# yongduosui/CAL

Measured on AMD Instinct MI355X. Metric: graphs/sec (train step) on SPMotif b=0.9 batch=128, higher is better.
Workload: dtype f32; 1 GPU; spmotif_b0.9_causalgcn_h128_l3_bs128; model=CausalGCN, batch_per_gpu=128, global_batch=128, hidden=128, layers=3, node_num=7, launch=graph(8 steps per graph launch, remainder 3), parallelism=dp1, resident_batches=8

## Files before the change

### cal_amd/csrc/engine.hip

```cpp
#include <string.h>
#include <hip/hip_ext.h>

#include <algorithm>
#include <type_traits>
#include <vector>

#include "engine_kernels.hpp"
#include "engine_readout.hpp"
#include "engine_gconv.hpp"
#include "engine_gconv_bwd.hpp"
#include "engine_ggat.hpp"
#include "engine_plan.hpp"
#include "engine_attbwd.hpp"
#include "engine_ro_step.hpp"
#include "engine_gin.hpp"
#include "engine_ggin.hpp"
#include "engine_feat.hpp"
#include "engine_gwide.hpp"
#include "engine_attwide.hpp"

namespace cal {

constexpr int MAX_LAYERS = 6;
constexpr int MAX_SLABS = 24;
// ... 1035 lines not shown
            { ProfScope ps(st, 0, 2.0 * N * H * H); RC(fwd_gemm(c, false, a, 1)); } STAGE();
            {
                ProfScope ps(st, 5, 2.0 * N * H * 4 + (double)(E + N) * (8 + 12.0 * K) + (N + 1) * 4.0);
                RC(gat_forward(e->rowptr_dst, e->nbr_dst, e->eid_dst, zi, e->P + e->o_conv_att[i - 1], e->P + e->o_conv_b[i - 1], 1,
                               e->gat_slope, c.training ? e->gat_p : 0.f, e->gat_seed[i - 1], (const uint64_t*)e->gat_ctr, hout,
                               sc, sc + nk, sc + 2 * nk, sc + 3 * nk, N, E, K, D, st));
            }
            STAGE();
            if (c.training && i < L) {
                int tc = std::min(256, pow2ceil(H));
                int rpb = std::max(32, cdiv(N, 1024));
                if (H == 256 && aligned16(hout))
                    hipLaunchKernelGGL(k_colstats4, dim3(cdiv(N, rpb)), dim3(256), 0, st, hout, N, rpb, Acc(bn_stsum(c, i + 1)), Acc(bn_stsq(c, i + 1)));
                else
                    hipLaunchKernelGGL(k_colstats, dim3(cdiv(N, rpb)), dim3(256), 0, st, hout, N, H, tc, rpb, Acc(bn_stsum(c, i + 1)), Acc(bn_stsq(c, i + 1)));
                CAL_CHECK_LAUNCH("k_colstats"); STAGE();
            }
        } else if (r.bb_fwd != Conv::Node) {
            GconvBranch gb;
            memset(&gb, 0, sizeof(gb));
            gb.x = hin; gb.W = e->P + e->o_conv_w[i - 1]; gb.bias = e->P + e->o_conv_b[i - 1];
            gb.dis = e->dis_unit; gb.bn = bnref(c, i, N, 1); gb.out = hout;
            if (i == 1 && !r.plan_coef) gb.coef_out = e->coef; else gb.coef_in = e->coef;
            if (c.training && i < L) { gb.st_sum = graph_acc(c, bn_stsum(c, i + 1), H, r.st_bb); gb.st_sq = graph_acc(c, bn_stsq(c, i + 1), H, r.st_bb); }
            const GconvBranch2 b2{{gb, gb}};
            {
                ProfScope ps(st, 2, 2.0 * N * H * H + 2.0 * (double)(E + N) * H, true);
                if (r.bb_fwd == Conv::Wide && r.gw_cols_bb == 32) PROF_LAUNCH((k_gw_fwd<false, 32>), dim3(T, H / 32, 1), dim3(GW_NT), 0, st, gd, e->gptr, e->eptr, b2, 1, e->loop_w, H, H, e->status);
                else if (r.bb_fwd == Conv::Wide) PROF_LAUNCH((k_gw_fwd<false, 64>), dim3(T, H / GC_N, 1), dim3(GW_NT), 0, st, gd, e->gptr, e->eptr, b2, 1, e->loop_w, H, H, e->status);
                else if (r.bb_fwd == Conv::Graph64) PROF_LAUNCH((k_gconv_fwd<false, 64, 512>), dim3(T, H / GC_N, 1), dim3(512), 0, st, gd, e->gptr, e->eptr, b2, 1, e->loop_w, H, H, e->status);
                else PROF_LAUNCH((k_gconv_fwd<false, GC_T>), dim3(T, H / GC_N, 1), dim3(256), 0, st, gd, e->gptr, e->eptr, b2, 1, e->loop_w, H, H, e->status);
            }
            CAL_CHECK_LAUNCH(r.bb_fwd == Conv::Wide ? "k_gw_fwd" : "k_gconv_fwd"); STAGE();
            RC(flush_finals(c)); STAGE();
        } else {
            GemmArgs a = gemm_args(N, H, H, false, false, 0);
            a.p[0].A = hin; a.p[0].B = e->P + e->o_conv_w[i - 1]; a.p[0].C = e->z;
            a.p[0].xa.has_bn = 1; a.p[0].xa.bn = bnref(c, i, N, 1);
            { ProfScope ps(st, 0, 2.0 * N * H * H); RC(fwd_gemm(c, false, a, 1)); } STAGE();
            SpmmBranch br{e->z, hout, e->P + e->o_conv_b[i - 1], nullptr, e->dis_unit, Acc(), Acc(), nullptr, nullptr, nullptr};
            const bool wst = c.training && i < L;
            const int rpb = spmm_rpb(H, wst, N);
            if (wst) { br.st_sum = spmm_acc(c, bn_stsum(c, i + 1), H, rpb); br.st_sq = spmm_acc(c, bn_stsq(c, i + 1), H, rpb); }
            {
                ProfScope ps(st, 1, 2.0 * N * H * 4 + (double)(E + N) * 8 + (N + 1) * 4.0, true);
                RC(launch_espmm(st, gd, SpmmBranch2{{br, br}}, 1, 1, e->loop_w, N, H, rpb));
            }
            CAL_CHECK_LAUNCH("k_espmm"); STAGE();
            RC(flush_finals(c)); STAGE();
        }
    }
    return 0;
}

int fwd_att(Ctx& c) {
    Engine* e = c.e;
    const Route& r = c.r;
    const int N = c.N, H = e->H, L = e->L;
    const int64_t E = c.E;
    hipStream_t st = c.st;
    const float* x = e->h + (size_t)L * N * H;
    const CSR gs = csr_src(c);
    if (r.att_fwd != Att::Node) {
        const bool wide = r.att_fwd == Att::Wide;
        const Acc a0 = graph_acc(c, bn_stsum(c, L + 1), H, r.st_co), a1 = graph_acc(c, bn_stsq(c, L + 1), H, r.st_co);
        const Acc a2 = graph_acc(c, bn_stsum(c, L + 2), H, r.st_co), a3 = graph_acc(c, bn_stsq(c, L + 2), H, r.st_co);
        auto launch = [&](auto kernel_of) {
            return with_g(H, [&](auto g) {
                hipLaunchKernelGGL(kernel_of(g), dim3(c.T), dim3(512), 0, st, e->gptr, gs, x, e->P + e->o_natt_w, e->P + e->o_natt_b,
                                   e->P + e->o_eatt_w, e->P + e->o_eatt_b, e->anode, e->pq, e->att, e->dis_co, e->dis_co + N, a0, a1, a2, a3,
                                   e->loop_w, H, E, e->status, e->no_node_att ? 0.f : 1.f, e->no_edge_att ? 0.f : 1.f, e->eptr);
                return 0;
            });
        };
        if (wide) RC(launch([](auto g) { return k_att_fwd_wide<4, decltype(g)::value>; }));
        else RC(launch([](auto g) { return k_att_fwd_graph<4, decltype(g)::value>; }));
        CAL_CHECK_LAUNCH(wide ? "k_att_fwd_wide" : "k_att_fwd_graph"); STAGE();
        RC(flush_finals(c)); STAGE();
        return 0;
    }
    const Acc a0 = node_acc(c, bn_stsum(c, L + 1), H), a1 = node_acc(c, bn_stsq(c, L + 1), H);
    const Acc a2 = node_acc(c, bn_stsum(c, L + 2), H), a3 = node_acc(c, bn_stsq(c, L + 2), H);
    RC(with_g(H, [&](auto g) {
        constexpr int G = decltype(g)::value;
        hipLaunchKernelGGL((k_node_att_fwd<4, G>), dim3(cdiv(N, c.rpb_n)), dim3(256), 0, st, x, e->P + e->o_natt_w,
                           e->P + e->o_natt_b, e->P + e->o_eatt_w, e->anode, e->pq, a0, a1, a2, a3, N, H, c.rpb_n, e->no_node_att ? 0.f : 1.f);
        return 0;
    }));
    CAL_CHECK_LAUNCH("k_node_att_fwd"); STAGE();
    RC(flush_finals(c)); STAGE();
    hipLaunchKernelGGL(k_edge_att_deg, dim3(cdiv(N, 32)), dim3(256), 0, st, gs, e->pq, e->P + e->o_eatt_b, e->att, e->dis_co,
                       e->dis_co + N, e->loop_w, N, E, e->no_edge_att ? 0.f : 1.f);
    CAL_CHECK_LAUNCH("k_edge_att_deg"); STAGE();
    return 0;
}

int fwd_co(Ctx& c) {
    Engine* e = c.e;
    const Route& r = c.r;
    const int N = c.N, B = c.B, T = c.T, H = e->H, L = e->L;
    const int64_t E = c.E;
    hipStream_t st = c.st;
    const size_t NH = (size_t)N * H;
    const float* x = e->h + (size_t)L * NH;
    const CSR gd = csr_dst(c);
    if (r.co_fwd != Conv::Node) {
        const bool wide = r.co_fwd == Conv::Wide;
        const int64_t* tgp = e->ntiles > 0 ? e->tile_gptr : nullptr;
        GconvBranch gb[2];
        memset(gb, 0, sizeof(gb));
        for (int k = 0; k < 2; ++k) {
            gb[k].x = x; gb[k].W = e->P + (k ? e->o_ow : e->o_cw); gb[k].bias = e->P + (k ? e->o_ob : e->o_cb);
            gb[k].ew = e->att + (size_t)k * E; gb[k].dis = e->dis_co + (size_t)k * N;
            gb[k].rs = e->anode + k; gb[k].rs_stride = 2; gb[k].bn = bnref(c, L + 1 + k, N, 1);
            gb[k].out = e->hco + (size_t)k * NH; gb[k].z = e->zco + (size_t)k * NH; gb[k].pooled = e->pooled + (size_t)k * B * H;
            if (wide) continue;
            gb[k].coef_out = e->coef + (size_t)(1 + k) * E;
            gb[k].w_out = e->wslot + (size_t)k * E;
            gb[k].batch = c.batch; gb[k].tile_gptr = tgp;
        }
        const GconvBranch2 b2{{gb[0], gb[1]}};
        if (tgp) hipLaunchKernelGGL((k_gconv_fwd<true, 64, 512, true>), dim3(T, H / GC_N, 2), dim3(512), 0, st, gd, e->gptr, e->eptr, b2, 1, e->loop_w, H, H, e->status);
        else if (r.co_fwd == Conv::Graph64) hipLaunchKernelGGL((k_gconv_fwd<true, 64, 512>), dim3(T, H / GC_N, 2), dim3(512), 0, st, gd, e->gptr, e->eptr, b2, 1, e->loop_w, H, H, e->status);
        else if (r.co_fwd == Conv::Graph128) hipLaunchKernelGGL((k_gconv_fwd<true, GC_T>), dim3(T, H / GC_N, 2), dim3(256), 0, st, gd, e->gptr, e->eptr, b2, 1, e->loop_w, H, H, e->status);
        else if (r.gw_cols_co == 32) hipLaunchKernelGGL((k_gw_fwd<true, 32>), dim3(T, H / 32, 2), dim3(GW_NT), 0, st, gd, e->gptr, e->eptr, b2, 1, e->loop_w, H, H, e->status);
        else hipLaunchKernelGGL((k_gw_fwd<true, 64>), dim3(T, H / GC_N, 2), dim3(GW_NT), 0, st, gd, e->gptr, e->eptr, b2, 1, e->loop_w, H, H, e->status);
        CAL_CHECK_LAUNCH(wide ? "k_gw_fwd(co)" : "k_gconv_fwd(co)"); STAGE();
        return 0;
    }
    GemmArgs a = gemm_args(N, H, H, false, false, 0);
    for (int k = 0; k < 2; ++k) {
        a.p[k].A = x; a.p[k].B = e->P + (k ? e->o_ow : e->o_cw); a.p[k].C = e->zco + (size_t)k * NH;
        a.p[k].xa.rs = e->anode + k; a.p[k].xa.rs_stride = 2;
        a.p[k].xa.has_bn = 1; a.p[k].xa.bn = bnref(c, L + 1 + k, N, 1);
    }
    RC(fwd_gemm(c, false, a, 2)); STAGE();
    SpmmBranch b0{e->zco, e->hco, e->P + e->o_cb, e->att, e->dis_co, Acc(), Acc(), nullptr, nullptr, nullptr};
    SpmmBranch b1{e->zco + NH, e->hco + NH, e->P + e->o_ob, e->att + E, e->dis_co + N, Acc(), Acc(), nullptr, nullptr, nullptr};
    RC(launch_espmm(st, gd, SpmmBranch2{{b0, b1}}, 2, 1, e->loop_w, N, H, spmm_rpb(H, false)));
    CAL_CHECK_LAUNCH("k_espmm(co)"); STAGE();
    RC(launch_pool2(c)); STAGE();
    return 0;
}

int fwd_readout(Ctx& c) {
    Engine* e = c.e;
    const int B = c.B, H = e->H, C = e->C, L = e->L;
    hipStream_t st = c.st;
    if (c.r.ro == Readout::OneLaunch || c.r.ro == Readout::Rows) {
        RoStepArgs sa;
        memset(&sa, 0, sizeof(sa));
        sa.a = make_ro(c); sa.zpart = e->zpart; sa.sync = reinterpret_cast<int*>(e->arena + e->a_sync); sa.status = e->status;
        if (c.r.ro == Readout::OneLaunch) {
            hipLaunchKernelGGL(k_ro_step<false>, dim3(3, H / RO_CW), dim3(256), 0, st, sa);
        } else {
            const int nrb = cdiv(B, RS_B), nch = H / RO_CW;
            sa.nrb = nrb;
            sa.xch = parts_alloc(c, (size_t)3 * nch * RBK_XCH);
            if (!sa.xch) return no_parts();
            sa.gw1_slab = e->slabs; sa.gw2_slab = e->slabs + (size_t)3 * nrb * H * H;
            hipLaunchKernelGGL(k_ro_step<true>, dim3(3, nch, nrb), dim3(256), 0, st, sa);
        }
        CAL_CHECK_LAUNCH("k_ro_step"); STAGE();
        return 0;
    }
    if (c.r.ro == Readout::FourKernel) {
        const RoArgs ra = make_ro(c);
        hipLaunchKernelGGL(k_ro_fwd_a, dim3(3, H / RO_CW), dim3(256), 0, st, ra);
        CAL_CHECK_LAUNCH("k_ro_fwd_a"); STAGE();
        hipLaunchKernelGGL(k_ro_fwd_b, dim3(3, cdiv(B, RO_RB)), dim3(256), 0, st, ra);
        CAL_CHECK_LAUNCH("k_ro_fwd_b"); STAGE();
        if (!c.want_grad) {
            hipLaunchKernelGGL(k_ro_loss, dim3(3), dim3(256), 0, st, ra);
            CAL_CHECK_LAUNCH("k_ro_loss");
        }
        return 0;
    }
    const int bn_fc1 = L + 3, bn_fc2 = L + 4;
    {
        int tc = std::min(256, pow2ceil(H));
        hipLaunchKernelGGL(k_readout_prep, dim3(cdiv(B, c.rpb_b)), dim3(256), 0, st, e->pooled, c.perm, e->iperm, e->xco, B, H, tc,
                           c.rpb_b, bn_stsum(c, bn_fc1), bn_stsq(c, bn_fc1), bn_stsum(c, bn_fc1 + 2), bn_stsq(c, bn_fc1 + 2),
                           bn_stsum(c, bn_fc1 + 4), bn_stsq(c, bn_fc1 + 4), e->cat);
        CAL_CHECK_LAUNCH("k_readout_prep"); STAGE();
    }
    const float* xin[3] = {e->pooled, e->pooled + (size_t)B * H, e->xco};
    const int Wco = e->cat ? 2 * H : H;
    {
        auto fc1 = [&](int hd0, int nh, int Kin) -> int {
            GemmArgs a = gemm_args(B, H, Kin, false, true, 1);
            for (int q = 0; q < nh; ++q) {
                const int hd = hd0 + q;
                a.p[q].A = xin[hd]; a.p[q].B = e->P + e->o_fc1_w[hd]; a.p[q].bias = e->P + e->o_fc1_b[hd];
                a.p[q].C = e->y1 + (size_t)hd * B * H;
                a.p[q].xa.has_bn = 1; a.p[q].xa.bn = bnref(c, bn_fc1 + 2 * hd, B, 1);
                if (c.training) gemm_stats(c, a.p[q], B, H, bn_stsum(c, bn_fc2 + 2 * hd), bn_stsq(c, bn_fc2 + 2 * hd), false);
            }
            return fwd_gemm(c, true, a, nh);
        };
        if (e->cat) { RC(fc1(0, 2, H)); STAGE(); RC(fc1(2, 1, Wco)); STAGE(); }
        else { RC(fc1(0, 3, H)); STAGE(); }
        RC(flush_finals(c)); STAGE();
    }
    {
        GemmArgs a = gemm_args(B, C, H, false, true, 0);
        for (int hd = 0; hd < 3; ++hd) {
            a.p[hd].A = e->y1 + (size_t)hd * B * H; a.p[hd].B = e->P + e->o_fc2_w[hd]; a.p[hd].bias = e->P + e->o_fc2_b[hd];
            a.p[hd].C = e->zl + (size_t)hd * B * C;
            a.p[hd].xa.has_bn = 1; a.p[hd].xa.bn = bnref(c, bn_fc2 + 2 * hd, B, 1);
        }
        RC(fwd_gemm(c, true, a, 3)); STAGE();
    }
    if (B > 256) hipLaunchKernelGGL(k_loss<1024>, dim3(1), dim3(1024), 0, st, e->zl, c.y, e->logp, e->dzl, e->stats, e->arena + e->a_db2, B, C, c.wc, c.wo,
                                    c.wco, c.want_grad);
    else hipLaunchKernelGGL(k_loss<256>, dim3(1), dim3(256), 0, st, e->zl, c.y, e->logp, e->dzl, e->stats, e->arena + e->a_db2, B, C, c.wc, c.wo,
                            c.wco, c.want_grad);
    CAL_CHECK_LAUNCH("k_loss"); STAGE();
    return 0;
}

int engine_forward(Ctx& c, const float* x0, const int64_t* edge_index) {
    RC(fwd_plan(c, x0, edge_index));
    RC(fwd_feat(c, x0));
    RC(fwd_backbone(c));
    RC(fwd_att(c));
    RC(fwd_co(c));
    return fwd_readout(c);
}

int bwd_readout(Ctx& c, Bwd& b) {
    Engine* e = c.e;
    const int B = c.B, H = e->H, C = e->C, L = e->L;
    const size_t BH = (size_t)B * H;
    hipStream_t st = c.st;
    FinishArgs& fa = b.fa;
    if (c.r.ro == Readout::Rows) {
        const int nrb = cdiv(B, RS_B);
        for (int hd = 0; hd < 3; ++hd) {
            fa.st[fa.nst++] = SlabTask{e->slabs + (size_t)hd * nrb * H * H, e->G + e->o_fc1_w[hd], H * H, nrb};
            fa.st[fa.nst++] = SlabTask{e->slabs + (size_t)3 * nrb * H * H + (size_t)hd * nrb * C * H, e->G + e->o_fc2_w[hd], C * H, nrb};
        }
        b.slab_off = (size_t)3 * nrb * ((size_t)H * H + (size_t)C * H);
        b.slab_off = (b.slab_off + 63) & ~(size_t)63;
    }
    if (c.r.ro != Readout::Gemm) {
        if (c.r.ro == Readout::FourKernel) {
            const RoArgs ra = make_ro(c);
            hipLaunchKernelGGL(k_ro_bwd_a, dim3(3, H / RO_CW), dim3(256), 0, st, ra);
            CAL_CHECK_LAUNCH("k_ro_bwd_a"); STAGE();
            hipLaunchKernelGGL(k_ro_bwd_b, dim3(3, H / RO_CW), dim3(256), 0, st, ra);
            CAL_CHECK_LAUNCH("k_ro_bwd_b"); STAGE();
        }
        fa.stats = e->stats; fa.wc = c.wc; fa.wo = c.wo; fa.wco = c.wco;
        return 0;
    }
    const int bn_fc1 = L + 3, bn_fc2 = L + 4;
    const float* xin[3] = {e->pooled, e->pooled + BH, e->xco};
    {
        GemmArgs a = gemm_args(C, H, B, true, false, 0);
        float* dst[3];
        for (int hd = 0; hd < 3; ++hd) {
            a.p[hd].A = e->dzl + (size_t)hd * B * C; a.p[hd].B = e->y1 + hd * BH;
            a.p[hd].xb.has_bn = 1; a.p[hd].xb.bn = bnref(c, bn_fc2 + 2 * hd, B, 0);
            dst[hd] = e->G + e->o_fc2_w[hd];
        }
        RC(grad_gemm(c, b, a, 3, dst)); STAGE();
    }
    {
        GemmArgs a = gemm_args(B, H, C, false, false, 0);
        for (int hd = 0; hd < 3; ++hd) {
            a.p[hd].A = e->dzl + (size_t)hd * B * C; a.p[hd].B = e->P + e->o_fc2_w[hd]; a.p[hd].C = e->dyh1 + hd * BH;
            a.p[hd].aux = e->y1 + hd * BH; a.p[hd].has_aux = 1; a.p[hd].aux_bn = bnref(c, bn_fc2 + 2 * hd, B, 0);
            gemm_stats(c, a.p[hd], B, H, bn_dsum(c, bn_fc2 + 2 * hd), bn_dprod(c, bn_fc2 + 2 * hd), true);
        }
        RC(fwd_gemm(c, false, a, 3)); STAGE();
        RC(flush_finals(c)); STAGE();
    }
    {
        BnBwdProb p[3];
        for (int hd = 0; hd < 3; ++hd)
            p[hd] = BnBwdProb{e->dyh1 + hd * BH, e->y1 + hd * BH, e->dy1 + hd * BH, bnref(c, bn_fc2 + 2 * hd, B, 0),
                              bn_dsum(c, bn_fc2 + 2 * hd), bn_dprod(c, bn_fc2 + 2 * hd), e->arena + e->a_db1 + hd * H};
        RC(with_g(H, [&](auto g) {
            constexpr int G = decltype(g)::value;
            hipLaunchKernelGGL((k_bn_bwd<4, G>), dim3(cdiv(B, c.rpb_b), 3), dim3(256), 0, st, BnBwdProb3{{p[0], p[1], p[2]}}, 1, B, H, c.rpb_b);
            return 0;
        }));
        CAL_CHECK_LAUNCH("k_bn_bwd(readout)"); STAGE();
    }
    const int Wco = e->cat ? 2 * H : H;
    float* const dxh_hd[3] = {e->dxh, e->dxh + BH, e->dxh + 2 * BH};
    {
        auto r4 = [&](int hd0, int nh, int Kin) -> int {
            GemmArgs a = gemm_args(H, Kin, B, true, false, 0);
            float* dst[3];
            for (int q = 0; q < nh; ++q) {
                const int hd = hd0 + q;
                a.p[q].A = e->dy1 + hd * BH; a.p[q].B = xin[hd];
                a.p[q].xb.has_bn = 1; a.p[q].xb.bn = bnref(c, bn_fc1 + 2 * hd, B, 0);
                dst[q] = e->G + e->o_fc1_w[hd];
            }
            return grad_gemm(c, b, a, nh, dst);
        };
        if (e->cat) { RC(r4(0, 2, H)); STAGE(); RC(r4(2, 1, Wco)); STAGE(); }
        else { RC(r4(0, 3, H)); STAGE(); }
    }
    {
// ... 903 lines not shown
```

### cal_amd/csrc/engine_ro_step.hpp

```cpp
#pragma once
#include "engine_readout.hpp"

namespace cal {

constexpr int RS_B = 128;
constexpr int RS_K = 128;
constexpr int RS_LD = RS_K + 4;

struct RoStepArgs {
    RoArgs a;
    float* zpart;
    int* sync;
    int* status;
    double* xch;
    float* gw1_slab; float* gw2_slab;
    int nrb;
};
constexpr int RBK_MAXRB = 4;
constexpr int RBK_N0 = 2 * RS_K, RBK_N1 = 2 * RO_CW, RBK_N2 = 2 * (RO_CW + 1), RBK_N3 = 4 * 64;
constexpr int RBK_O1 = RBK_MAXRB * RBK_N0, RBK_O2 = RBK_O1 + RBK_MAXRB * RBK_N1, RBK_O3 = RBK_O2 + RBK_MAXRB * RBK_N2;
constexpr int RBK_XCH = RBK_O3 + RBK_MAXRB * RBK_N3;
constexpr int RBK_SYNC_INTS = 3 * RBK_MAXRB * 2 + 3 * (RS_K / RO_CW) * 4;

__device__ __forceinline__ void ro_step_arrive(int* ctr) {
    __syncthreads();
    if (threadIdx.x == 0) __hip_atomic_fetch_add(ctr, 1, __ATOMIC_RELEASE, __HIP_MEMORY_SCOPE_AGENT);
}
__device__ __forceinline__ void ro_step_wait(int* ctr, int n, int* status) {
    if (threadIdx.x == 0) {
        int spins = 0;
        while (__hip_atomic_load(ctr, __ATOMIC_RELAXED, __HIP_MEMORY_SCOPE_AGENT) < n) {
            if (++spins > (1 << 21)) { if (status) atomicOr(status, 256); break; }
            __builtin_amdgcn_s_sleep(1);
        }
        __builtin_amdgcn_fence(__ATOMIC_ACQUIRE, "agent");
    }
    __syncthreads();
}
__device__ __forceinline__ void ro_step_barrier(int* ctr, int n, int* status) {
    ro_step_arrive(ctr);
    ro_step_wait(ctr, n, status);
}
template <int NT, bool BN>
__device__ __forceinline__ void ro_mfma_rowk_nt(int kred, const float* X, int ld, int nrow, const float* Wr, const float* sc,
                                                const float* sh, ro_f32x4 (&acc)[4]) {
    const int l = threadIdx.x & 63, w = threadIdx.x >> 6, lr = l & 15, lk = l >> 4;
    const float* ar[NT];
#pragma unroll
    for (int t = 0; t < NT; ++t) ar[t] = X + min((w + 4 * t) * 16 + lr, nrow - 1) * ld + 4 * lk;
    const float* br = Wr + lr * ld + 4 * lk;
    float4 a4[NT], b4, s4 = make_float4(1.f, 1.f, 1.f, 1.f), h4 = make_float4(0.f, 0.f, 0.f, 0.f);
    auto fetch = [&](int k0, float4 (&a)[NT], float4& b, float4& s, float4& h) {
#pragma unroll
        for (int t = 0; t < NT; ++t) a[t] = *reinterpret_cast<const float4*>(ar[t] + k0);
        b = *reinterpret_cast<const float4*>(br + k0);
        if (BN) { s = *reinterpret_cast<const float4*>(sc + k0 + 4 * lk); h = *reinterpret_cast<const float4*>(sh + k0 + 4 * lk); }
    };
    fetch(0, a4, b4, s4, h4);
    for (int k0 = 0; k0 < kred; k0 += 16) {
        float4 an[NT], bn, sn = s4, hn = h4;
        fetch(min(k0 + 16, kred - 16), an, bn, sn, hn);
        const float bb[4] = {b4.x, b4.y, b4.z, b4.w}, ss[4] = {s4.x, s4.y, s4.z, s4.w}, hh[4] = {h4.x, h4.y, h4.z, h4.w};
#pragma unroll
        for (int j = 0; j < 4; ++j)
#pragma unroll
            for (int t = 0; t < NT; ++t) {
                const float aa[4] = {a4[t].x, a4[t].y, a4[t].z, a4[t].w};
                acc[t] = __builtin_amdgcn_mfma_f32_16x16x4f32(BN ? fmaf(aa[j], ss[j], hh[j]) : aa[j], bb[j], acc[t], 0, 0, 0);
            }
#pragma unroll
        for (int t = 0; t < NT; ++t) a4[t] = an[t];
        b4 = bn; s4 = sn; h4 = hn;
    }
}
template <bool BN>
__device__ __forceinline__ void ro_mfma_rowk(int ntiles, int kred, const float* X, int ld, int nrow, const float* Wr, const float* sc,
                                             const float* sh, ro_f32x4 (&acc)[4]) {
    switch ((ntiles + 3) / 4) {
        case 1: ro_mfma_rowk_nt<1, BN>(kred, X, ld, nrow, Wr, sc, sh, acc); break;
        case 2: ro_mfma_rowk_nt<2, BN>(kred, X, ld, nrow, Wr, sc, sh, acc); break;
        case 3: ro_mfma_rowk_nt<3, BN>(kred, X, ld, nrow, Wr, sc, sh, acc); break;
        default: ro_mfma_rowk_nt<4, BN>(kred, X, ld, nrow, Wr, sc, sh, acc); break;
    }
}

template <int NV>
__device__ __forceinline__ void rbk_total(double (&v)[NV], int t, int n, double* xs, int nrb, int rb, int* ctr, int* status) {
    if (t < n) {
#pragma unroll
        for (int q = 0; q < NV; ++q) xs[(size_t)rb * NV * n + q * n + t] = v[q];
    }
    ro_step_barrier(ctr, nrb, status);
    if (t < n) {
#pragma unroll
        for (int q = 0; q < NV; ++q) {
            double tot = 0.0;
            for (int r = 0; r < nrb; ++r) tot += xs[(size_t)r * NV * n + q * n + t];
            v[q] = tot;
        }
    }
}

template <bool RBK>
__global__ void __launch_bounds__(256) k_ro_step(const RoStepArgs sa) {
    warm_kernargs<(sizeof(RoStepArgs) < 1024 ? sizeof(RoStepArgs) : 1024)>();
    const RoArgs& a = sa.a;
    __shared__ __attribute__((aligned(16))) float Xs[RS_B * RS_LD];
    __shared__ __attribute__((aligned(16))) float Ws[RO_CW * RS_LD];
    __shared__ __attribute__((aligned(16))) float W1t[RO_CW * RS_LD];
    __shared__ __attribute__((aligned(16))) float scratch[2 * RS_B * RO_CW];
    __shared__ __attribute__((aligned(16))) float xn[RS_B * RO_CW];
    __shared__ __attribute__((aligned(16))) float y1c[RS_B * RO_CW];
    __shared__ __attribute__((aligned(16))) float zs[2048];
    __shared__ __attribute__((aligned(16))) float W2c[64 * RO_CW];
    __shared__ __attribute__((aligned(16))) float sc_s[RS_K], sh_s[RS_K], mean1_s[RS_K], rstd1_s[RS_K];
    __shared__ int perm_s[256];
    __shared__ double red[2][256];
    __shared__ float c2[6][RO_CW];
    __shared__ double lossp_s[2];
    const int hd = blockIdx.x, ch = blockIdx.y, j0 = ch * RO_CW, nch = gridDim.y;
    const int Bt = a.B, rb = RBK ? (int)blockIdx.z : 0, r0 = rb * RS_B, nrb = RBK ? sa.nrb : 1;
    const int B = RBK ? min(RS_B, Bt - r0) : Bt, K = a.H, C = a.C, ld = RS_LD, K4 = K / 4, BC = B * C, BCt = Bt * C;
    int* const cbar = RBK ? sa.sync + (hd * RBK_MAXRB + rb) * 2 : sa.sync + hd * 2;
    int* const gbar = sa.sync + 3 * RBK_MAXRB * 2 + (hd * nch + ch) * 4;
    double* const xch = RBK ? sa.xch + (size_t)(hd * nch + ch) * RBK_XCH : nullptr;
    const RoHead& h = a.h[hd];
    const int l = threadIdx.x & 63, w = threadIdx.x >> 6, j = l & 15, lk = l >> 4;
    const int rl = threadIdx.x / RO_CW;
    float* dyh = scratch;
    float* yn = scratch + RS_B * RO_CW;
    double (*red8)[256] = reinterpret_cast<double (*)[256]>(scratch);
    const int B16 = (B + 15) & ~15, ntiles = B16 / 16;
    const bool duty_out = ch == 1 % nch, duty_loss = ch == 2 % nch, duty_db2 = ch == 3 % nch,
               duty_xco = ch == 4 % nch, duty_run1 = ch == 5 % nch;

    RO_CLK(40);
    const bool colfix = 256 % K4 == 0;
    float sf[4] = {0.f, 0.f, 0.f, 0.f}, qf[4] = {0.f, 0.f, 0.f, 0.f}, pvt[4] = {0.f, 0.f, 0.f, 0.f};
    int nst = 0;
    auto add_stats = [&](const float4 v) {
        const float vv[4] = {v.x, v.y, v.z, v.w};
#pragma unroll
        for (int c = 0; c < 4; ++c) {
            pvt[c] = nst == 0 ? vv[c] : pvt[c];
            const float d = vv[c] - pvt[c];
            sf[c] += d; qf[c] = fmaf(d, d, qf[c]);
        }
        ++nst;
    };
    int pv = hd == 2 ? (int)a.perm[r0 + min((int)threadIdx.x, B - 1)] : 0;
    float g2 = h.bn2.gamma[j0 + j], b2n = h.bn2.beta[j0 + j], rm2 = h.bn2.run_mean[j0 + j], rv2 = h.bn2.run_var[j0 + j];
    float bias1 = h.b1[j0 + j];
    float rm1 = h.bn1.run_mean[min((int)threadIdx.x, K - 1)], rv1 = h.bn1.run_var[min((int)threadIdx.x, K - 1)];
    int ylab = (int)a.y[r0 + min((int)threadIdx.x, B - 1)];
    {
        RoBatch<float4, 2> bw;
        RoBatch<float, 8> bt;
        RoBatch<float, 4> bw2;
        ro_issue(bw, RO_CW, K4, [&](int jj, int c) { return *reinterpret_cast<const float4*>(h.W1 + (size_t)(j0 + jj) * K + c * 4); });
        ro_issue(bt, K, RO_CW, [&](int jj, int ii) { return h.W1[(size_t)jj * K + j0 + ii]; });
        ro_issue(bw2, C, RO_CW, [&](int c, int jj) { return h.W2[(size_t)c * K + j0 + jj]; });
        auto commit_weights = [&]() {
            ro_commit(bw, RO_CW, K4, [&](int jj, int c, const float4 v) { *reinterpret_cast<float4*>(Ws + jj * ld + c * 4) = v; });
            ro_commit(bt, K, RO_CW, [&](int jj, int ii, float v) { W1t[ii * ld + jj] = v; });
            ro_commit(bw2, C, RO_CW, [&](int c, int jj, float v) { W2c[c * RO_CW + jj] = v; });
            asm volatile("" : "+v"(g2), "+v"(b2n), "+v"(rm2), "+v"(rv2), "+v"(bias1), "+v"(ylab), "+v"(rm1), "+v"(rv1));
        };
        RoBatch<float4, 16> bx;
        if (hd == 2) {
            asm volatile("" : "+v"(pv));
            perm_s[threadIdx.x] = pv;
            __syncthreads();
            RoBatch<float4, 16> bp;
            ro_issue(bx, B, K4, [&](int b, int c) { return *reinterpret_cast<const float4*>(a.pooled + (size_t)(Bt + r0 + b) * K + c * 4); });
            ro_issue(bp, B, K4, [&](int b, int c) { return *reinterpret_cast<const float4*>(a.pooled + (size_t)perm_s[b] * K + c * 4); });
            commit_weights();
            ro_commit2(bx, bp, B, K4, [&](int b, int c, const float4 o, const float4 p) {
                const float4 v = make_float4(p.x + o.x, p.y + o.y, p.z + o.z, p.w + o.w);
                *reinterpret_cast<float4*>(Xs + b * ld + c * 4) = v;
                if (colfix) add_stats(v);
                if (duty_xco) *reinterpret_cast<float4*>(a.xco + (size_t)(r0 + b) * K + c * 4) = v;
            });
            if (duty_xco && (int)threadIdx.x < B) a.iperm[pv] = r0 + threadIdx.x;
        } else {
            const float* src = a.pooled + (hd == 0 ? (size_t)0 : (size_t)Bt * K) + (size_t)r0 * K;
            ro_issue(bx, B, K4, [&](int b, int c) { return *reinterpret_cast<const float4*>(src + (size_t)b * K + c * 4); });
            commit_weights();
            ro_commit(bx, B, K4, [&](int b, int c, const float4 v) {
                *reinterpret_cast<float4*>(Xs + b * ld + c * 4) = v;
                if (colfix) add_stats(v);
            });
        }
        __syncthreads();
    }
    RO_CLK(41);
    {
        const int np = 256 / K4, cg = threadIdx.x % K4, part = threadIdx.x / K4;
        if (!colfix && part < np) {
#pragma unroll 4
            for (int b = part; b < B; b += np) add_stats(*reinterpret_cast<const float4*>(Xs + b * ld + 4 * cg));
        }
#pragma unroll
        for (int c = 0; c < 4; ++c) {
            const double P = (double)pvt[c], S0 = (double)sf[c], n0 = (double)nst;
            red8[c][threadIdx.x] = S0 + n0 * P;
            red8[4 + c][threadIdx.x] = (double)qf[c] + 2.0 * P * S0 + n0 * P * P;
        }
        __syncthreads();
        double SQ[2] = {0.0, 0.0};
        if ((int)threadIdx.x < K) {
            const int g = threadIdx.x >> 2, c = threadIdx.x & 3;
            for (int p = 0; p < np; ++p) { SQ[0] += red8[c][p * K4 + g]; SQ[1] += red8[4 + c][p * K4 + g]; }
        }
        if (RBK) rbk_total<2>(SQ, threadIdx.x, K, xch, nrb, rb, gbar + 0, sa.status);
        if ((int)threadIdx.x < K) {
            const int k = threadIdx.x;
            const double S = SQ[0], Q = SQ[1];
            float sc, sh, mean, rstd;
            ro_bn_from_sums(h.bn1, k, S, Q, sc, sh, mean, rstd);
            sc_s[k] = sc; sh_s[k] = sh; mean1_s[k] = mean; rstd1_s[k] = rstd;
            if (duty_run1 && rb == 0) {
                const double m = S * (double)h.bn1.inv_n;
                double v = Q * (double)h.bn1.inv_n - m * m;
                if (v < 0.0) v = 0.0;
                h.bn1.run_mean[k] = 0.9f * rm1 + 0.1f * (float)m;
                h.bn1.run_var[k] = 0.9f * rv1 + 0.1f * (float)(v * (double)h.bn1.unbias);
                if (k == 0 && h.bn1.nbt) *h.bn1.nbt += 1;
            }
        }
        __syncthreads();
    }
    RO_CLK(42);
    for (int idx = threadIdx.x; idx < B16 * RO_CW; idx += 256) {
        const int b = idx / RO_CW, ii = idx % RO_CW;
        xn[idx] = b < B ? Xs[b * ld + j0 + ii] : 0.f;
    }
    ro_f32x4 acc[4] = {};
    ro_mfma_rowk<true>(ntiles, K, Xs, ld, B, Ws, sc_s, sh_s, acc);
    float s1 = 0.f, s2 = 0.f, pv2 = 0.f;
    int n2 = 0;
#pragma unroll
    for (int t = 0; t < 4; ++t)
#pragma unroll
        for (int r = 0; r < 4; ++r) {
            const int b = (w + 4 * t) * 16 + lk * 4 + r;
            const float v = b < B ? fmaxf(acc[t][r] + bias1, 0.f) : 0.f;
            if (b < B) y1c[b * RO_CW + j] = v;
            pv2 = (b < B && n2 == 0) ? v : pv2;
            const float d = b < B ? v - pv2 : 0.f;
            n2 += b < B ? 1 : 0;
            s1 += d; s2 = fmaf(d, d, s2);
        }
    RO_CLK(43);
    {
        const double P = (double)pv2, S0 = (double)s1, n0 = (double)n2;
        red[0][threadIdx.x] = S0 + n0 * P; red[1][threadIdx.x] = (double)s2 + 2.0 * P * S0 + n0 * P * P;
    }
// ... 27 lines not shown
        float* zp = sa.zpart + ((size_t)hd * nch + ch) * BCt + (size_t)r0 * C;
        for (int o = threadIdx.x; o < BC; o += 256) {
            const int b = o / C, c = o % C;
            const float4* yr = reinterpret_cast<const float4*>(yn + b * RO_CW);
            const float4* wr = reinterpret_cast<const float4*>(W2c + c * RO_CW);
            zp[o] = dot4(yr[3], wr[3], dot4(yr[2], wr[2], dot4(yr[1], wr[1], dot4(yr[0], wr[0], 0.f))));
        }
    }
    RO_CLK(44);
    ro_step_barrier(cbar, nch, sa.status);
    RO_CLK(45);

    for (int o0 = 0; o0 < BC; o0 += 512) {
        float pz[2][8], bz[2];
#pragma unroll
        for (int v = 0; v < 2; ++v) {
            const int o = min(o0 + v * 256 + (int)threadIdx.x, BC - 1);
            bz[v] = h.b2[o % C];
#pragma unroll
            for (int p = 0; p < 8; ++p) pz[v][p] = sa.zpart[((size_t)hd * nch + min(p, nch - 1)) * BCt + (size_t)r0 * C + o];
        }
#pragma unroll
        for (int v = 0; v < 2; ++v) {
            ro_pin(bz[v]);
#pragma unroll
            for (int p = 0; p < 8; ++p) ro_pin(pz[v][p]);
        }
#pragma unroll
        for (int v = 0; v < 2; ++v) {
            const int o = o0 + v * 256 + (int)threadIdx.x;
            float z = 0.f;
#pragma unroll
            for (int p = 0; p < 8; ++p) z += p < nch ? pz[v][p] : 0.f;
            z += bz[v];
            if (o < BC) {
                zs[o] = z;
                if (duty_out) a.zl[(size_t)hd * BCt + (size_t)r0 * C + o] = z;
            }
        }
    }
    __syncthreads();
    float lv = 0.f, cv = 0.f;
    if ((int)threadIdx.x < B) {
        const int b = threadIdx.x;
        const float u = 1.0f / (float)C, invB = 1.0f / (float)Bt, logu = logf(u);
        const float wgt = hd == 0 ? a.wc : (hd == 1 ? a.wo : a.wco);
        float* zr = zs + b * C;
        const int yy = ylab;
        int arg = 0; float best = -INFINITY;
        double lrow = 0.0;
        auto finish = [&](int k, float zk, float lse) {
            const float lp = zk - lse;
            if (lp > best) { best = lp; arg = k; }
            if (hd == 0) lrow += (double)(u * (logu - lp));
            else if (k == yy) lrow = (double)(-lp);
            const float p = expf(lp);
            const float dz = wgt * invB * (hd == 0 ? (p - u) : (p - (k == yy ? 1.f : 0.f)));
            zr[k] = dz;
            if (duty_out) { a.logp[(size_t)hd * BCt + (size_t)(r0 + b) * C + k] = lp; a.dzl[(size_t)hd * BCt + (size_t)(r0 + b) * C + k] = dz; }
        };
        if (C <= 8) {
            float zc[8];
#pragma unroll
            for (int k = 0; k < 8; ++k) zc[k] = zr[min(k, C - 1)];
            float m = zc[0];
#pragma unroll
            for (int k = 1; k < 8; ++k) m = fmaxf(m, zc[k]);
            float se = 0.f;
#pragma unroll
            for (int k = 0; k < 8; ++k) se += k < C ? expf(zc[k] - m) : 0.f;
            const float lse = m + logf(se);
#pragma unroll
            for (int k = 0; k < 8; ++k) if (k < C) finish(k, zc[k], lse);
        } else {
            float m = -INFINITY;
            for (int k = 0; k < C; ++k) m = fmaxf(m, zr[k]);
            float se = 0.f;
            for (int k = 0; k < C; ++k) se += expf(zr[k] - m);
            const float lse = m + logf(se);
            for (int k = 0; k < C; ++k) finish(k, zr[k], lse);
        }
        lv = (float)lrow; cv = arg == yy ? 1.f : 0.f;
    }
    if (duty_loss) {
        double ls = (double)lv, cs = (double)cv;
#pragma unroll
        for (int o = 32; o > 0; o >>= 1) { ls += __shfl_xor(ls, o, 64); cs += __shfl_xor(cs, o, 64); }
        if (l == 0) { red[0][w] = ls; red[1][w] = cs; }
        __syncthreads();
        if (threadIdx.x == 0) {
            const double lsum = red[0][0] + red[0][1] + red[0][2] + red[0][3], csum = red[1][0] + red[1][1] + red[1][2] + red[1][3];
            if (RBK) { lossp_s[0] = lsum; lossp_s[1] = csum; }
            else {
                a.stats[1 + hd] = (float)(lsum / (double)Bt);
                a.stats[hd == 1 ? 4 : (hd == 0 ? 5 : 6)] = (float)csum;
            }
        }
    }
    __syncthreads();
    RO_CLK(46);
    const float* dzs = zs;
    double db1_keep = 0.0, db2_keep = 0.0;
    {
        float t1f = 0.f, t2f = 0.f;
        float dq[8] = {0.f, 0.f, 0.f, 0.f, 0.f, 0.f, 0.f, 0.f};
        for (int c = 0; c < C; ++c) {
            const float wc2 = W2c[c * RO_CW + j];
            float dzv[8];
#pragma unroll
            for (int qq = 0; qq < 8; ++qq) dzv[qq] = dzs[min(rl + 16 * qq, B - 1) * C + c];
#pragma unroll
            for (int qq = 0; qq < 8; ++qq) dq[qq] = fmaf(dzv[qq], wc2, dq[qq]);
        }
#pragma unroll
        for (int qq = 0; qq < 8; ++qq) {
            const int b = rl + 16 * qq;
            const float yv = y1c[min(b, B - 1) * RO_CW + j];
            if (b < B) {
                const float n = (yv - mean2) * rstd2;
                dyh[b * RO_CW + j] = dq[qq];
                t1f += dq[qq]; t2f = fmaf(dq[qq], n, t2f);
            }
        }
        double t1 = (double)t1f, t2 = (double)t2f;
        red[0][threadIdx.x] = t1; red[1][threadIdx.x] = t2;
        __syncthreads();
        if (rl == 0) for (int p = 1; p < 16; ++p) { t1 += red[0][p * RO_CW + j]; t2 += red[1][p * RO_CW + j]; }
        if (RBK) {
            double tt[2] = {rl == 0 ? t1 : 0.0, rl == 0 ? t2 : 0.0};
            if (threadIdx.x == RO_CW) { tt[0] = duty_loss ? lossp_s[0] : 0.0; tt[1] = duty_loss ? lossp_s[1] : 0.0; }
            rbk_total<2>(tt, threadIdx.x, RO_CW + 1, xch + RBK_O2, nrb, rb, gbar + 2, sa.status);
            t1 = tt[0]; t2 = tt[1];
            if (threadIdx.x == RO_CW && duty_loss && rb == 0) {
                a.stats[1 + hd] = (float)(tt[0] / (double)Bt);
                a.stats[hd == 1 ? 4 : (hd == 0 ? 5 : 6)] = (float)tt[1];
            }
        }
        if (rl == 0) {
            if (rb == 0) { h.d2_sum[j0 + j] = t1; h.d2_prod[j0 + j] = t2; }
            c2[4][j] = (float)(t1 * (double)h.bn2.inv_n); c2[5][j] = (float)(t2 * (double)h.bn2.inv_n);
        }
        __syncthreads();
        const float m1 = c2[4][j], m2 = c2[5][j], gs = gam2 * rstd2;
        float sbf = 0.f;
#pragma unroll
        for (int qq = 0; qq < 8; ++qq) {
            const int b = rl + 16 * qq;
            if (b < B) {
                const float yv = y1c[b * RO_CW + j];
                const float n = (yv - mean2) * rstd2;
                const float dy = yv > 0.f ? gs * (dyh[b * RO_CW + j] - m1 - n * m2) : 0.f;
                a.dy1[((size_t)hd * Bt + r0 + b) * K + j0 + j] = dy;
                sbf += dy;
            }
        }
        double sb = (double)sbf;
        red[0][threadIdx.x] = sb;
        __syncthreads();
        if (rl == 0) {
            for (int p = 1; p < 16; ++p) sb += red[0][p * RO_CW + j];
            if (RBK) db1_keep = sb; else h.db1[j0 + j] = sb;
        }
    }
    RO_CLK(47);
    ro_step_arrive(cbar + 1);
    RO_CLK(48);
    ro_step_wait(cbar + 1, nch, sa.status);
    RO_CLK(49);
    float* Ds = Xs;
    RoBatch<float4, 16> bd;
    ro_issue(bd, B, K4, [&](int b, int c) { return *reinterpret_cast<const float4*>(a.dy1 + ((size_t)hd * Bt + r0 + b) * K + c * 4); });
    if (duty_db2) {
        const int np = 256 / C, c = threadIdx.x % C, part = threadIdx.x / C;
        double sdz = 0.0;
        if (part < np) for (int b = part; b < B; b += np) sdz += (double)dzs[b * C + c];
        red[0][threadIdx.x] = sdz;
        __syncthreads();
        if (part == 0) {
            for (int p2 = 1; p2 < np; ++p2) sdz += red[0][p2 * C + c];
            if (RBK) db2_keep = sdz; else h.db2[c] = sdz;
        }
        __syncthreads();
    }
    {
        const int nout = C * RO_CW;
        float* fred = dyh;
        for (int o0 = 0; o0 < nout; o0 += 256) {
            const int no = min(256, nout - o0), np = 256 / no;
            const int o = o0 + threadIdx.x % no, part = threadIdx.x / no;
            const int c = o / RO_CW, jj = o % RO_CW;
            float accw = 0.f;
            if (part < np) {
#pragma unroll 4
                for (int b = part; b < B; b += np) accw = fmaf(dzs[b * C + c], yn[b * RO_CW + jj], accw);
            }
            __syncthreads();
            fred[threadIdx.x] = accw;
            __syncthreads();
            if (part == 0) {
                for (int p = 1; p < np; ++p) accw += fred[p * no + threadIdx.x];
                (RBK ? sa.gw2_slab + ((size_t)hd * nrb + rb) * C * K : h.gW2)[(size_t)c * K + j0 + jj] = accw;
            }
        }
    }
    ro_commit(bd, B, K4, [&](int b, int c, const float4 v) { *reinterpret_cast<float4*>(Ds + b * ld + c * 4) = v; });
    for (int idx = threadIdx.x; idx < (B16 - B) * ld; idx += 256) Ds[B * ld + idx] = 0.f;
    __syncthreads();
    RO_CLK(50);
    const int i = j, i0 = j0;
    const float mean1 = mean1_s[i0 + i], rstd1 = rstd1_s[i0 + i], gs1 = sc_s[i0 + i], sh1 = sh_s[i0 + i];
    ro_f32x4 dacc[4] = {};
    ro_mfma_rowk<false>(ntiles, K, Ds, ld, B, W1t, nullptr, nullptr, dacc);
    float u1 = 0.f, u2 = 0.f;
#pragma unroll
    for (int t = 0; t < 4; ++t)
#pragma unroll
        for (int r = 0; r < 4; ++r) {
            const int b = (w + 4 * t) * 16 + lk * 4 + r;
            const float n = (xn[min(b, B16 - 1) * RO_CW + i] - mean1) * rstd1;
            const float dv = b < B ? dacc[t][r] : 0.f;
            u1 += dv; u2 = fmaf(dv, n, u2);
        }
    red[0][threadIdx.x] = (double)u1; red[1][threadIdx.x] = (double)u2;
    __syncthreads();
    {
        double uu[4] = {0.0, 0.0, 0.0, 0.0};
        if (threadIdx.x < RO_CW)
            for (int p = 0; p < 16; ++p) { uu[0] += red[0][p * RO_CW + threadIdx.x]; uu[1] += red[1][p * RO_CW + threadIdx.x]; }
        if (RBK) {
            uu[2] = threadIdx.x < RO_CW ? db1_keep : 0.0;
            uu[3] = (duty_db2 && (int)threadIdx.x < C) ? db2_keep : 0.0;
            rbk_total<4>(uu, threadIdx.x, 64, xch + RBK_O3, nrb, rb, gbar + 3, sa.status);
            if (rb == 0) {
                if (threadIdx.x < RO_CW) h.db1[j0 + threadIdx.x] = uu[2];
                if (duty_db2 && (int)threadIdx.x < C) h.db2[threadIdx.x] = uu[3];
            }
        }
        if (threadIdx.x < RO_CW) {
            const double S = uu[0], Q = uu[1];
            if (rb == 0) { h.d1_sum[i0 + threadIdx.x] = S; h.d1_prod[i0 + threadIdx.x] = Q; }
            c2[4][threadIdx.x] = (float)(S * (double)h.bn1.inv_n); c2[5][threadIdx.x] = (float)(Q * (double)h.bn1.inv_n);
        }
    }
    __syncthreads();
    {
        const float m1 = c2[4][i], m2 = c2[5][i];
#pragma unroll
        for (int t = 0; t < 4; ++t)
#pragma unroll
            for (int r = 0; r < 4; ++r) {
                const int b = (w + 4 * t) * 16 + lk * 4 + r;
                if (b < B) {
                    const float xr = xn[b * RO_CW + i];
                    const float n = (xr - mean1) * rstd1;
                    a.dxin[((size_t)hd * Bt + r0 + b) * K + i0 + i] = gs1 * (dacc[t][r] - m1 - n * m2);
                    xn[b * RO_CW + i] = fmaf(xr, gs1, sh1);
                }
            }
    }
    __syncthreads();
    RO_CLK(51);
    ro_f32x4 wacc[4] = {};
    ro_mfma_tiles(K / 16, B16, [&](int row, int k) { return Ds[k * ld + min(row, K - 1)]; },
                  [&](int k, int col) { return xn[k * RO_CW + col]; }, wacc);
#pragma unroll
    for (int t = 0; t < 4; ++t)
        if (w + 4 * t < K / 16) {
#pragma unroll
            for (int r = 0; r < 4; ++r)
                (RBK ? sa.gw1_slab + ((size_t)hd * nrb + rb) * K * K : h.gW1)[(size_t)((w + 4 * t) * 16 + lk * 4 + r) * K + i0 + i] = wacc[t][r];
        }
    RO_CLK(52);
}

}
```

Before: 606,300 graphs/s.

## Compute readout dW1 gradient early to overlap with the cross-block barrier wait

```diff
diff --git a/cal_amd/csrc/engine.hip b/cal_amd/csrc/engine.hip
--- a/cal_amd/csrc/engine.hip
+++ b/cal_amd/csrc/engine.hip
@@ -1211,7 +1211,7 @@
         memset(&sa, 0, sizeof(sa));
         sa.a = make_ro(c); sa.zpart = e->zpart; sa.sync = reinterpret_cast<int*>(e->arena + e->a_sync); sa.status = e->status;
         if (c.r.ro == Readout::OneLaunch) {
-            hipLaunchKernelGGL(k_ro_step<false>, dim3(3, H / RO_CW), dim3(256), 0, st, sa);
+            hipLaunchKernelGGL(k_ro_step<false>, dim3(RO_STEP_GX, H / RO_CW), dim3(256), 0, st, sa);
         } else {
             const int nrb = cdiv(B, RS_B), nch = H / RO_CW;
             sa.nrb = nrb;
diff --git a/cal_amd/csrc/engine_ro_step.hpp b/cal_amd/csrc/engine_ro_step.hpp
--- a/cal_amd/csrc/engine_ro_step.hpp
+++ b/cal_amd/csrc/engine_ro_step.hpp
@@ -2,6 +2,12 @@
 #include "engine_readout.hpp"
 
 namespace cal {
+
+#ifndef CAL_RO_PATH
+#define CAL_RO_PATH 0x01
+#endif
+constexpr bool RO_DW1_EARLY = (CAL_RO_PATH & 1) != 0, RO_HEAD_XCD = (CAL_RO_PATH & 4) != 0;
+constexpr int RO_STEP_GX = RO_HEAD_XCD ? 8 : 3;
 
 constexpr int RS_B = 128;
 constexpr int RS_K = 128;
@@ -84,6 +90,41 @@
     }
 }
 
+template <int NT>
+__device__ __forceinline__ void ro_mfma_dw1_nt(int B, int B16, int K, const float* X, int ld, const float* sc, const float* sh,
+                                               const float* dyc, ro_f32x4 (&acc)[4]) {
+    const int l = threadIdx.x & 63, w = threadIdx.x >> 6, lr = l & 15, lk = l >> 4;
+    int col[NT];
+    float scr[NT], shr[NT];
+#pragma unroll
+    for (int t = 0; t < NT; ++t) { col[t] = min((w + 4 * t) * 16 + lr, K - 1); scr[t] = sc[col[t]]; shr[t] = sh[col[t]]; }
+    auto fetch = [&](int k0, float (&bv)[4], float (&av)[4][NT]) {
+#pragma unroll
+        for (int j = 0; j < 4; ++j) {
+            const int k = k0 + 4 * j + lk;
+            bv[j] = dyc[k * RO_CW + lr];
+#pragma unroll
+            for (int t = 0; t < NT; ++t) av[j][t] = X[min(k, B - 1) * ld + col[t]];
+        }
+    };
+    float bv[4], av[4][NT];
+    fetch(0, bv, av);
+    for (int k0 = 0; k0 < B16; k0 += 16) {
+        float bn[4], an[4][NT];
+        fetch(min(k0 + 16, B16 - 16), bn, an);
+#pragma unroll
+        for (int j = 0; j < 4; ++j)
+#pragma unroll
+            for (int t = 0; t < NT; ++t) acc[t] = __builtin_amdgcn_mfma_f32_16x16x4f32(fmaf(av[j][t], scr[t], shr[t]), bv[j], acc[t], 0, 0, 0);
+#pragma unroll
+        for (int j = 0; j < 4; ++j) {
+            bv[j] = bn[j];
+#pragma unroll
+            for (int t = 0; t < NT; ++t) av[j][t] = an[j][t];
+        }
+    }
+}
+
 template <int NV>
 __device__ __forceinline__ void rbk_total(double (&v)[NV], int t, int n, double* xs, int nrb, int rb, int* ctr, int* status) {
     if (t < n) {
@@ -103,6 +144,7 @@
 
 template <bool RBK>
 __global__ void __launch_bounds__(256) k_ro_step(const RoStepArgs sa) {
+    if (!RBK && RO_HEAD_XCD && blockIdx.x >= 3) return;
     warm_kernargs<(sizeof(RoStepArgs) < 1024 ? sizeof(RoStepArgs) : 1024)>();
     const RoArgs& a = sa.a;
     __shared__ __attribute__((aligned(16))) float Xs[RS_B * RS_LD];
@@ -436,7 +478,8 @@
                 const float dy = yv > 0.f ? gs * (dyh[b * RO_CW + j] - m1 - n * m2) : 0.f;
                 a.dy1[((size_t)hd * Bt + r0 + b) * K + j0 + j] = dy;
                 sbf += dy;
-            }
+                if (RO_DW1_EARLY) y1c[b * RO_CW + j] = dy;
+            } else if (RO_DW1_EARLY && b < B16) y1c[b * RO_CW + j] = 0.f;
         }
         double sb = (double)sbf;
         red[0][threadIdx.x] = sb;
@@ -449,6 +492,13 @@
     RO_CLK(47);
     ro_step_arrive(cbar + 1);
     RO_CLK(48);
+    ro_f32x4 wacc[4] = {};
+    if (RO_DW1_EARLY) {
+        switch ((K / 16 + 3) / 4) {
+            case 1: ro_mfma_dw1_nt<1>(B, B16, K, Xs, ld, sc_s, sh_s, y1c, wacc); break;
+            default: ro_mfma_dw1_nt<2>(B, B16, K, Xs, ld, sc_s, sh_s, y1c, wacc); break;
+        }
+    }
     ro_step_wait(cbar + 1, nch, sa.status);
     RO_CLK(49);
     float* Ds = Xs;
@@ -489,6 +539,13 @@
     }
     ro_commit(bd, B, K4, [&](int b, int c, const float4 v) { *reinterpret_cast<float4*>(Ds + b * ld + c * 4) = v; });
     for (int idx = threadIdx.x; idx < (B16 - B) * ld; idx += 256) Ds[B * ld + idx] = 0.f;
+    if (RO_DW1_EARLY) {
+        float* gw = (RBK ? sa.gw1_slab + ((size_t)hd * nrb + rb) * K * K : h.gW1) + (size_t)(j0 + j) * K + lk * 4;
+#pragma unroll
+        for (int t = 0; t < 2; ++t)
+            if (w + 4 * t < K / 16)
+                *reinterpret_cast<float4*>(gw + (w + 4 * t) * 16) = make_float4(wacc[t][0], wacc[t][1], wacc[t][2], wacc[t][3]);
+    }
     __syncthreads();
     RO_CLK(50);
     const int i = j, i0 = j0;
@@ -538,13 +595,13 @@
                     const float xr = xn[b * RO_CW + i];
                     const float n = (xr - mean1) * rstd1;
                     a.dxin[((size_t)hd * Bt + r0 + b) * K + i0 + i] = gs1 * (dacc[t][r] - m1 - n * m2);
-                    xn[b * RO_CW + i] = fmaf(xr, gs1, sh1);
+                    if (!RO_DW1_EARLY) xn[b * RO_CW + i] = fmaf(xr, gs1, sh1);
                 }
             }
     }
+    if (RO_DW1_EARLY) { RO_CLK(51); RO_CLK(52); return; }
     __syncthreads();
     RO_CLK(51);
-    ro_f32x4 wacc[4] = {};
     ro_mfma_tiles(K / 16, B16, [&](int row, int k) { return Ds[k * ld + min(row, K - 1)]; },
                   [&](int k, int col) { return xn[k * RO_CW + col]; }, wacc);
 #pragma unroll
```

After: 609,800 graphs/s, median of 6. About the same (+0.6%).
